# fakufaku/diffusion-separation

Hardware: AMD Instinct MI355X
Metric: separated utterances/sec (4 s, 8 kHz, 2-spk, N=30 PC steps) (higher is better)
Workload: dtype f16; 1 GPU; configs[1]: 2-spk N=30 PC sampler (+1 ald2 corrector step), batch=16 x 4.0 s @ 8 kHz per GPU and step, NCSN++ nf=64 random-init, 60 NFE/step; 4 consecutive steps (batches) in flight per GPU; batch_per_gpu=16, samples=32000, N=30, corrector_steps=1, nf=64, graph=True, batches_in_flight=4

## Files before the change

diffusion-separation_amd/csrc/common.h:

```cpp
#pragma once
#include <hip/hip_runtime.h>
#include <stdint.h>
#include <stdio.h>

#include <string>

typedef uint16_t bf16_t;
typedef __attribute__((ext_vector_type(16))) float f32x16;
typedef __attribute__((ext_vector_type(8))) __bf16 bf16x8;

#define DS_F32 0
#define DS_BF16 1
#define DS_F32_SPLIT 2
#define DS_MAX_SRC 4

void ds_set_error(const std::string& s);
#define DS_CHECK(cond, msg)                                                            \
  do {                                                                                 \
    if (!(cond)) {                                                                     \
      ds_set_error(std::string(__FILE__) + ":" + std::to_string(__LINE__) + ": " + (msg)); \
      return 1;                                                                        \
    }                                                                                  \
  } while (0)
#define DS_HIP(expr)                                                                   \
// ... 157 lines not shown
  const void* sw; int sw_chunked;
  const float* gn_scale;
  const float* gn_shift; int gn_act;
  const float* bias;
  const float* bias_b; int bias_b_ld;
  int bias_mode;
  const float* div_b;
  const void* res; long res_bs; int ldr;
  float out_scale;
  void* y; long y_bs; int ldy;
  long long* stats_acc;
  const long long* gn_acc1; const long long* gn_acc2; const float* gn_gamma; const float* gn_beta;
  int gn_groups; float gn_inv_count; float gn_eps;
  int B, H, W;
  int Cin, Cout, taps;
  int dtype;
  int split;
  unsigned opts;
};
#define DS_OPT_NO_RW 1u
#define DS_OPT_NO_RW128 2u
#define DS_OPT_RW_SMALL 4u
#define DS_OPT_NO_RW_RES 8u
#define DS_OPT_NO_ATTN_FUSED 64u
#define DS_OPT_NO_SPLIT256 128u
#define DS_OPT_NO_STFT_FUSED 256u
#define DS_OPT_RW_QUARTER 1024u
#define DS_OPT_RW_BIG_HALF 2048u
#define DS_OPT_RW_HALF 512u
#define DS_OPT_NO_SW 4096u
#define DS_OPT_NO_SW_RW 8192u
#define DS_OPT_NO_SW_ROWS4 32768u
#define DS_OPT_SW_ROWS4 65536u
#define DS_OPT_NO_SWS 16384u
#define DS_OPT_NO_WFRAG 32u
unsigned ds_default_opts();
int ds_num_cus();
enum { DS_CLS_CONV_N64 = 0, DS_CLS_CONV_N32, DS_CLS_CONV_8X8, DS_CLS_GEMM_N64, DS_CLS_GEMM_N32, DS_CLS_GEMM_8X8, DS_CLS_WS,
       DS_CLS_SMALL, DS_CLS_RW, DS_CLS_ATTN, DS_CLS_SW, DS_CLS_SWS, DS_NCLS };
enum class ConvRoute { GENERIC, WS, THIN_IN, THIN_OUT, SMALL, RW, SW, SWS };
struct ConvPlan {
  ConvRoute route;
  int cls;
  int tile;
  int sw_rows;
  bool rw_ok;
  bool skip_ok;
};
ConvPlan ds_conv_plan(const ConvArgs& a);
int ds_launch_conv(const ConvArgs& a, hipStream_t st);
int ds_launch_conv(const ConvArgs& a, const ConvPlan& p, hipStream_t st);
const char* ds_last_conv_kernel();
void ds_set_last_conv_kernel(const char* name);
int ds_conv_chunk(int taps, int dtype);
__host__ __device__ inline long ds_rw_frag_index(int co, int tap, int ch, int taps, int Cout) {
  return (((((long)(ch / 64) * taps + tap) * 4 + (ch % 64) / 16) * (Cout / 32) + co / 32) * 64 + ((ch % 16) / 8) * 32 + co % 32) * 8 + ch % 8;
}
inline bool ds_rw_frag_shape(int taps, int Cin, int Cout) {
  return (Cout == 64 || Cout == 128) && (Cin == 64 || Cin == 128) && (taps == 1 || !(Cout == 128 && Cin == 64));
}
bool ds_conv_rw_supported(const ConvArgs& a);
int ds_launch_conv_rw(const ConvArgs& a, hipStream_t st);
inline bool ds_sw_frag_shape(int taps, int Cin, int Cout) { return (Cout == 64 || Cout == 128 || Cout == 256) && Cin % 64 == 0 && Cin >= 64 && Cin <= 512; }
bool ds_conv_sw_supported(const ConvArgs& a);
int ds_launch_conv_sw(const ConvArgs& a, int rows, hipStream_t st);
__host__ __device__ inline long ds_sws_frag_index(int co, int tap, int ch, int taps, int Cout, int plane) {
  return ((((((long)(ch / 32) * taps + tap) * 2 + (ch % 32) / 16) * 2 + plane) * (Cout / 32) + co / 32) * 64 + ((ch % 16) / 8) * 32 + co % 32) * 8 + ch % 8;
}
inline bool ds_sws_frag_shape(int taps, int Cin, int Cout) { return (Cout == 64 || Cout == 128 || Cout == 256) && Cin % 64 == 0 && Cin >= 64 && Cin <= 256; }
bool ds_conv_sws_supported(const ConvArgs& a);
int ds_launch_conv_sws(const ConvArgs& a, hipStream_t st);
bool ds_conv_ws_supported(const ConvArgs& a);
int ds_launch_conv_ws(const ConvArgs& a, hipStream_t st);
bool ds_conv_thin_in_supported(const ConvArgs& a);
int ds_launch_conv_thin_in(const ConvArgs& a, hipStream_t st);
bool ds_conv_thin_out_supported(const ConvArgs& a);
int ds_launch_conv_thin_out(const ConvArgs& a, hipStream_t st);
bool ds_conv_small_supported(const ConvArgs& a);
int ds_launch_conv_small(const ConvArgs& a, hipStream_t st);

struct AttnFusedArgs {
  const void* x; long x_bs; int ldx;
  const long long* gn_acc; const float* gn_gamma; const float* gn_beta; int gn_groups; float gn_inv_count; float gn_eps;
  const float* gn_scale; const float* gn_shift;
  const void* wqk; const void* wv; const void* wo;
// ... 147 lines not shown
```

diffusion-separation_amd/csrc/conv3x3_halo.h:

```cpp
#pragma once

#include <ctype.h>
#include <stdlib.h>

#include <initializer_list>
#include <type_traits>

#include "conv_device.h"

#ifdef HALO_TIMING
#define HALO_CAT_(a, b, c) a##b##c
#define HALO_CAT(a, b, c) HALO_CAT_(a, b, c)
#define HALO_DBG HALO_CAT(g_, HALO_TIMING, _dbg)
__device__ unsigned long long HALO_DBG[16];
extern "C" int HALO_CAT(diffsep_, HALO_TIMING, _debug_read)(unsigned long long* out, int reset) {
  (void)hipMemcpyFromSymbol(out, HIP_SYMBOL(HALO_DBG), sizeof(unsigned long long) * 16);
  if (reset) { unsigned long long z[16] = {0}; (void)hipMemcpyToSymbol(HIP_SYMBOL(HALO_DBG), z, sizeof(z)); }
  return 0;
}
#define RT_DECL unsigned rt_prev = (unsigned)__builtin_readcyclecounter(), rt_acc[8] = {0, 0, 0, 0, 0, 0, 0, 0};
#define RT_MARK(i) { unsigned rt_now = (unsigned)__builtin_readcyclecounter(); rt_acc[i] += rt_now - rt_prev; rt_prev = rt_now; }
#define RT_FLUSH if (threadIdx.x == 0) { for (int q = 0; q < 8; ++q) atomicAdd(&HALO_DBG[q], (unsigned long long)rt_acc[q]); atomicAdd(&HALO_DBG[15], 1ull); }
#define HALO_STR_(a) #a
#define HALO_STR(a) HALO_STR_(a)
// ... 66 lines not shown
    k.sx2 = reinterpret_cast<const T*>(a.sx2); k.sx2_bs = a.sx2_bs; k.ldsx2 = a.sx2 ? a.ldsx2 : a.ldsx;
    k.swfrag = reinterpret_cast<const bf16_t*>(a.sw_frag);
    return a.sCin;
  }
  if (a.res) {
    k.sx = reinterpret_cast<const T*>(a.res); k.sx_bs = a.res_bs; k.ldsx = a.ldr; k.sC1 = a.Cout; k.ldsx2 = a.ldr;
    k.swfrag = reinterpret_cast<const bf16_t*>(a.ident_frag);
    return a.Cout;
  }
  return 0;
}

inline int halo_tiles(const ConvArgs& a, int tile_h) { return (a.H / tile_h) * (a.W / TW); }
inline int halo_blocks_wanted(const ConvArgs& a, int ncb) {
  const int g = ds_num_cus() / (a.B * ncb);
#ifdef HALO_TIMING
  return halo_env("G", g);
#else
  return g;
#endif
}
template <auto KERN, typename K>
int halo_launch(K k, const ConvArgs& a, int tile_h, int g, int ncb, int lds, hipStream_t st, const char* family,
                std::initializer_list<int> targs) {
  const int tiles = halo_tiles(a, tile_h);
  k.G = g < 1 ? 1 : (g > tiles ? tiles : g);
  k.tiles_x = a.W / TW;
  k.tiles_per_img = tiles;
  DS_FUNC_LDS_ONCE(KERN, lds);
  hipLaunchKernelGGL(KERN, dim3(a.B * ncb * k.G), dim3(NT), lds, st, k);
  DS_LAUNCH_CHECK();
  static char name[64] = {0};
  if (!name[0]) {
    char b[64];
    int n = snprintf(b, sizeof(b), "%s<", family);
    for (int v : targs) n += snprintf(b + n, sizeof(b) - n, "%d,", v);
    b[n - 1] = '>';
    for (int i = n; i >= 0; --i) name[i] = b[i];
  }
  ds_set_last_conv_kernel(name);
  return 0;
}

inline bool halo_concat_ok(const ConvArgs& a, int kc, int al) {
  return a.x2 ? a.C1 % kc == 0 && a.C1 > 0 && a.C1 < a.Cin && a.ldx % al == 0 && a.ldx2 % al == 0 : a.ldx % al == 0;
}
inline bool halo_gn_ok(const ConvArgs& a, int cpg_max) {
  if ((a.gn_scale || a.gn_acc1) && !a.gn_act) return false;
  return !a.gn_acc1 || (a.gn_groups > 0 && a.Cin % a.gn_groups == 0 && a.Cin / a.gn_groups <= cpg_max && (!a.x2 || a.gn_acc2));
}
inline bool halo_skip_split_ok(const ConvArgs& a, int kc, int al) {
  return a.ldsx % al == 0 && (!a.sx2 || (a.sC1 % kc == 0 && a.sC1 > 0 && a.sC1 < a.sCin && a.ldsx2 % al == 0));
}
// ... 16 lines not shown
```

diffusion-separation_amd/csrc/conv3x3_rw.hip:

```cpp
#include <stdlib.h>

#ifdef RW_TIMING
#define HALO_TIMING rw
#endif
#include "conv3x3_halo.h"

namespace {

constexpr int KC = 64;
constexpr int NKB = KC / 16;
constexpr int KSC = 9 * NKB;
static_assert(KC * 2 + 16 == AROW && KC / 8 == PPL, "a pixel's chunk is one 128-byte line");

struct RwK {
  const bf16_t* x; long x_bs; int ldx; int C1;
  const bf16_t* x2; long x2_bs; int ldx2;
  const bf16_t* w; int w_chunked;
  const bf16_t* wfrag; const bf16_t* swfrag;
  const float* gn_scale; const float* gn_shift;
  const long long* gn_acc1; const long long* gn_acc2; const float* gn_gamma; const float* gn_beta;
  int gn_groups; float gn_inv_count; float gn_eps;
  const float* bias; const float* bias_b; int bias_b_ld;
  const bf16_t* res; long res_bs; int ldr;
  float out_scale;
  bf16_t* y; long y_bs; int ldy;
  long long* stats;
  const bf16_t* sx; long sx_bs; int ldsx; int sC1;
  const bf16_t* sx2; long sx2_bs; int ldsx2;
  const bf16_t* sw; int sw_chunked; int sw_shift; int sCin;
  int H, W, G, tiles_x, tiles_per_img;
  int dbg;
};

#ifndef RW_NWL2
#define RW_NWL2 8
#endif
constexpr int rw_lds_ksteps(int nch, int rpw, int nsk, int ncg) { return ncg == 4 ? nch * KSC - 64 + nsk * NKB : (nch == 2 ? RW_NWL2 : 0); }

template <int NCH, int RPW, int NSK, int NCG>
struct RwGeom {
  static constexpr int CO = 32 * NCG, PGN = 4 / NCG;
  static constexpr int TH = PGN * RPW, HH_ = TH + 2, HP = HH_ * HW_;
  static constexpr int NI = TH * TW * PPL / NT, NBP = HP - TH * TW, NB = (NBP * PPL + NT - 1) / NT;
  static constexpr int NL = NI + NB;
  static_assert(NT / PPL == TW && TH * TW * PPL % NT == 0, "one staging pass = one tile row");
  static constexpr int LDS_A = NL * (NT / PPL) * AROW;
  static constexpr int CIN = NCH * KC, SCIN = NSK * KC;
  static constexpr int LDS_TAB = (2 * CIN + CO) * 4;
  static constexpr int LDS_DESC = NB * NT * 4;
  static_assert((NI + NB) * (NT / PPL) >= HP + NB * (NT / PPL) - NBP, "dummy pixels of the last border pass fit the slot");
  static constexpr int NPH = NCH + NSK;
  static constexpr int NKS = NCH * KSC + NSK * NKB;
  static constexpr int NWL = rw_lds_ksteps(NCH, RPW, NSK, NCG), NWR = NKS - NWL;
  static constexpr int LDS_WL = NWL * NCG * 64 * 16;
  static constexpr int WL_STEP = NCG * 64 * 16;
  static constexpr int OFF_TAB = 2 * LDS_A, OFF_WL = OFF_TAB + ((LDS_TAB + 15) & ~15), OFF_DESC = OFF_WL + LDS_WL;
  static constexpr int LDS_TOTAL = OFF_DESC + LDS_DESC;
  static constexpr int chunk_of(int P) { return P < NSK ? NCH + P : P - NSK; }
  static_assert(LDS_TOTAL <= 160 * 1024, "LDS budget of one CU");
  static_assert(NT * 36 * 4 <= LDS_TOTAL, "the statistics reduce reuses the block's LDS");
};

template <int NCH, int RPW, int NSK, int MODE, int NCG>
__global__ __launch_bounds__(NT, 1) void conv3x3_rw_kernel(RwK p) {
  using G = RwGeom<NCH, RPW, NSK, NCG>;
  constexpr int CO = G::CO, PGN = G::PGN;
  constexpr int TH = G::TH, HP = G::HP, LDS_A = G::LDS_A, NL = G::NL, NPH = G::NPH, NKS = G::NKS, CIN = G::CIN, NWR = G::NWR;
  extern __shared__ __attribute__((aligned(16))) char smem[];
  char* sA = smem;
  float* sTab = reinterpret_cast<float*>(smem + G::OFF_TAB);
  int* sDesc = reinterpret_cast<int*>(smem + G::OFF_DESC);
  const int tid = threadIdx.x;
  const int lane = tid & 63, wave = __builtin_amdgcn_readfirstlane(tid >> 6);
  const int l32 = lane & 31, h = lane >> 5;
  const int cg = wave % NCG, pg = wave / NCG;
  const int b = blockIdx.x / p.G, part = blockIdx.x % p.G;
  const int t0 = (int)((long)part * p.tiles_per_img / p.G);
  const int nt = (int)((long)(part + 1) * p.tiles_per_img / p.G) - t0;
  RT_DECL

  static_assert(CIN <= NT && CO <= NT, "one table entry per thread");
  constexpr int CPG_MAX = 8;
  long long t_s[CPG_MAX], t_q[CPG_MAX];
  float t_gam = 1.f, t_bet = 0.f, t_sc = 1.f, t_sh = 0.f, t_bias = 0.f;
#pragma unroll
  for (int j = 0; j < CPG_MAX; ++j) { t_s[j] = 0; t_q[j] = 0; }
  if (tid < CIN) {
    const int c = tid;
    if (p.gn_acc1) {
      const int C1 = p.C1, C2 = CIN - C1;
      const int cpg = CIN / p.gn_groups, g0 = (c / cpg) * cpg;
#pragma unroll
      for (int j = 0; j < CPG_MAX; ++j) {
        if (j < cpg) {
          const int cc = g0 + j;
          const long long* src = cc < C1 ? p.gn_acc1 + ((long)b * C1 + cc) * 2 : p.gn_acc2 + ((long)b * C2 + (cc - C1)) * 2;
          t_s[j] = src[0];
          t_q[j] = src[1];
        }
      }
      t_gam = p.gn_gamma ? p.gn_gamma[c] : 1.f;
      t_bet = p.gn_beta ? p.gn_beta[c] : 0.f;
    } else if (p.gn_scale) {
      t_sc = p.gn_scale[(long)b * CIN + c];
      t_sh = p.gn_shift[(long)b * CIN + c];
    }
  }
  if (tid < CO) t_bias = (p.bias ? p.bias[tid] : 0.f) + (p.bias_b ? p.bias_b[(long)b * p.bias_b_ld + tid] : 0.f);
  auto build_tables = [&]() __attribute__((always_inline)) {
    if (tid < CIN) {
      float sc = t_sc, sh = t_sh;
      if (p.gn_acc1) {
        long long t_ssum = 0, t_ssq = 0;
#pragma unroll
        for (int j = 0; j < CPG_MAX; ++j) { t_ssum += t_s[j]; t_ssq += t_q[j]; }
        ds_gn_affine_from_acc(t_ssum, t_ssq, p.gn_inv_count, p.gn_eps, t_gam, t_bet, sc, sh);
      }
      sTab[tid] = sc;
      sTab[CIN + tid] = sh;
    }
    if (tid < CO) sTab[2 * CIN + tid] = t_bias * p.out_scale;
  };
  const int slot = tid & (PPL - 1);
  constexpr int NI = G::NI, NB = G::NB, NBP = G::NBP;
  const int ixp = tid / PPL;
  unsigned fl = 0;
  int dstb[NB];
#pragma unroll
  for (int kb = 0; kb < NB; ++kb) {
    const int bi = ixp + (NT / PPL) * kb;
    int hy, hx;
// ... 206 lines not shown
#else
      if (P1 < NCH || k < NI)
        *reinterpret_cast<u32x4_t*>(sA + sl * LDS_A + (k < NI ? ldi0 + k * HW_ * AROW : dstb[k < NI ? 0 : k - NI])) = so;
#endif
#ifdef RW_ABL_NOLOAD
      pa[k][0] += rel;
#else
      issue_one(P2_, g2, k, rel);
#endif
    }
  };
  auto unit_s2 = [&](auto P1_, auto P2_, const TileG& g1, const TileG& g2, int sl, int u, int rel) __attribute__((always_inline)) {
    unit_s2x(P1_, P2_, std::false_type{}, g1, g2, sl, u, rel);
  };
  auto unit_fin = [&](auto P1_, auto P2_, const TileG& g1, const TileG& g2, int sl, int u, int rel) __attribute__((always_inline)) {
    unit_s2x(P1_, P2_, std::true_type{}, g1, g2, sl, u, rel);
  };
  auto unit = [&](auto P1_, auto P2_, const TileG& g1, const TileG& g2, int sl, int u, int rel) __attribute__((always_inline)) {
    unit_s01(P1_, u, -1);
    unit_s01(P1_, -1, u);
    unit_s2(P1_, P2_, g1, g2, sl, u, rel);
  };

  f32x16 acc[RPW];
#pragma unroll
  for (int r = 0; r < RPW; ++r)
#pragma unroll
    for (int e = 0; e < 16; ++e) acc[r][e] = 0.f;
  float ssum[16], ssq[16];
#pragma unroll
  for (int j = 0; j < 16; ++j) { ssum[j] = 0.f; ssq[j] = 0.f; }
  const bool has_stats = p.stats != nullptr;
  const float osc = FOLD ? p.out_scale * -0.6931471805599453f : p.out_scale;
  const int fbase = (pg * RPW * HW_ + l32) * AROW + h * 16;

  auto swap_halves = [&](u32x4_t& v) __attribute__((always_inline)) {
    auto r0 = __builtin_amdgcn_permlane32_swap(v.x, v.z, false, false);
    auto r1 = __builtin_amdgcn_permlane32_swap(v.y, v.w, false, false);
    v.x = r0[0]; v.z = r0[1]; v.y = r1[0]; v.w = r1[1];
  };
  u32x4_t ov0;
  const int srow = lane >> 4;
  const unsigned spiece = (unsigned)(cg * 64 + (srow & 1) * 32 + (srow >> 1) * 16);
  auto epi_unit = [&](const TileG& g, int r, int j, const float4& t0, const float4& t1) __attribute__((always_inline)) {
    float v[8];
    v[0] = fmaf(acc[r][8 * j + 0], osc, t0.x); v[1] = fmaf(acc[r][8 * j + 1], osc, t0.y);
// ... 58 lines not shown
  auto half = [&](auto P_, auto HF_, auto EPI_, int slot_r, const TileG& ge, const TileG& g1, const TileG& g2) __attribute__((always_inline)) {
    constexpr int P = decltype(P_)::value, HF = decltype(HF_)::value;
    constexpr bool EPI = decltype(EPI_)::value;
    constexpr int C = G::chunk_of(P);
    constexpr bool CONV = C < NCH;
    constexpr int NK = CONV ? KSC : NKB;
    constexpr int W0 = CONV ? C * KSC : NCH * KSC + (C - NCH) * NKB;
    constexpr int C1 = G::chunk_of((P + 1) % NPH), C2 = G::chunk_of((P + 2) % NPH);
    constexpr int NU = NL * 4;
    constexpr bool ACT1 = C1 < NCH && MODE != 0;
    constexpr int LAG = ACT1 ? PIPE_LAG : 0, NUV = NU + LAG, NLU = 2 * NUV;
    constexpr int NGH = NK * RH;
    constexpr int w0 = (P == 0) ? W_E : W_N, w1 = (P == NPH - 1) ? W_E : W_N, CAP = NGH * (w0 + w1);
    auto lub = [](int GP) constexpr { return NLU * (GP <= NGH ? GP * w0 : NGH * w0 + (GP - NGH) * w1) / CAP; };
    constexpr int NLE = RH * 22;
    constexpr int R0 = HF * RH, ER0 = HF ? 0 : RH;
    const char* fb = sA + slot_r * LDS_A + fbase + R0 * HW_ * AROW;
#ifndef RW_BUILTIN_MFMA
    if constexpr (EPI) {
#pragma unroll
      for (int r = 0; r < RH; ++r) asm volatile("s_nop 11" : "+v"(acc[ER0 + r]));
    }
#endif
    if constexpr (HF == 0 && C1 < NCH) act_tab(C1);
    constexpr int SUB = CONV ? 3 : 1, RFN = CONV ? RH + 2 : RH, NG = NK / SUB;
    static_assert(SUB * RH >= RFN, "the next group's fragments are read in the MFMA slots of the current one");
    auto ldg = [&](int g, int j) __attribute__((always_inline)) {
      const int dx = CONV ? g / NKB : 1, kb = g % NKB, row = CONV ? j : j + 1;
      return *reinterpret_cast<const u32x4_t*>(fb + (row * HW_ + dx) * AROW + kb * 32);
    };
    u32x4_t rf[2][RFN];
#pragma unroll
    for (int j = 0; j < RFN; ++j) rf[0][j] = ldg(0, j);
    auto widx = [](int ks) {
      if (!CONV) return ks;
      const int g = ks / 3, dy = ks % 3, dx = g / NKB, kb = g % NKB;
      return (dy * 3 + dx) * NKB + kb;
    };
#define RW_FRAG(ks, r) rf[((ks) / SUB) & 1][(r) + (CONV ? (ks) % SUB : 0)]
#define RW_FRAG_LAST(ks) rf[((ks) / SUB) & 1][RFN - 1]
    u32x4_t wl = {0, 0, 0, 0}, wln = {0, 0, 0, 0};
    if constexpr (W0 + widx(0) >= NWR) wl = *reinterpret_cast<const u32x4_t*>(sWl + (W0 + widx(0) - NWR) * G::WL_STEP);
    int rels[2][NL];
    auto fetch_rels = [&](int ks, int par) __attribute__((always_inline)) {
      const int gp0 = HF * NGH + ks * RH;
#pragma unroll
      for (int L = lub(gp0); L < lub(gp0 + RH); ++L) {
        const int u = (L >> 1) - LAG;
        if ((L & 1) && u >= 0 && u < NU && (u & 3) == 3 && (u >> 2) >= NI)
          rels[par][u >> 2] = REL_REGS ? relreg[(u >> 2) - NI] : sDesc[((u >> 2) - NI) * NT + tid];
      }
    };
    fetch_rels(0, 0);

    auto unit_lump = [&](int L, int par) __attribute__((always_inline)) {
      const int v = L >> 1;
      const int u0 = v < NU ? v : -1, u1 = LAG ? ((v >= 1 && v - 1 < NU) ? v - 1 : -1) : v, u2 = v - LAG;
      const bool s2 = u2 >= 0 && u2 < NU;
      if ((L & 1) == 0) {
        if constexpr (ACT1 && ACT_PK) {
          if (u0 >= 0) {
            asm volatile("v_pk_fma_f16 %0, %1, %2, %3" : "=v"(uzp[u0 % 3]) : "v"(pa[u0 >> 2][u0 & 3]), "v"(psc[u0 & 3]), "v"(psh[u0 & 3]));
            if constexpr (MODE == 2 && !FOLD) asm volatile("v_pk_mul_f16 %0, %1, %2" : "=v"(uxp[u0 % 3]) : "v"(uzp[u0 % 3]), "s"(0xbdc5bdc5u));
          }
          if constexpr (MODE == 2) {
            if (u1 >= 0) asm volatile("v_pk_add_f16 %0, %1, %2" : "=v"(udp[u1 % 3]) : "v"(utp[u1 % 3]), "s"(0x3c003c00u));
            if (s2) asm volatile("v_pk_mul_f16 %0, %1, %2" : "=v"(so[u2 & 3]) : "v"(uzp[u2 % 3]), "v"(urp[u2 % 3]));
            if (u0 >= 0) asm volatile("v_exp_f16 %0, %1" : "=v"(utp[u0 % 3]) : "v"(FOLD ? uzp[u0 % 3] : uxp[u0 % 3]));
            if (u1 >= 0) asm volatile("v_rcp_f16 %0, %1" : "=v"(urp[u1 % 3]) : "v"(udp[u1 % 3]));
          } else {
            if (s2) so[u2 & 3] = uzp[u2 % 3];
          }
        } else if constexpr (ACT1) {
          if (u0 >= 0) unit_s01(std::integral_constant<int, C1>{}, u0, -1);
        }
      } else {
// ... 52 lines not shown
        }
      } else if (x == 20) {
#pragma unroll
        for (int d = 0; d < 4; ++d) asm volatile("v_permlane16_swap_b32 %0, %1" : "+v"(osa[d]), "+v"(osb[d]));
      } else {
        const int pix = ge.pix0 + (pg * RPW + rr) * p.W + (lane & 15);
        const unsigned o = __umul24((unsigned)pix, (unsigned)p.ldy * 2u) + spiece;
#ifdef RW_TIMING
        const unsigned o1 = (p.dbg & 1) ? OOB : o, o2 = (p.dbg & 1) ? OOB : o + 16u * (unsigned)p.ldy * 2u;
#else
        const unsigned o1 = o, o2 = o + 16u * (unsigned)p.ldy * 2u;
#endif
#ifdef RW_ABL_NOSTORE
        asm volatile("" :: "v"(osa), "v"(osb), "v"(o1), "v"(o2));
#else
        __builtin_amdgcn_raw_buffer_store_b128(osa, ry, o1, 0, 0);
        __builtin_amdgcn_raw_buffer_store_b128(osb, ry, o2, 0, 0);
#endif
      }
    };

#pragma unroll
    for (int ks = 0; ks < NK; ++ks) {
      if (ks + 1 < NK) fetch_rels(ks + 1, (ks + 1) & 1);
      const int wi = W0 + widx(ks), win = W0 + widx(ks + 1 < NK ? ks + 1 : ks);
      if (win >= NWR && ks + 1 < NK) wln = *reinterpret_cast<const u32x4_t*>(sWl + (win - NWR) * G::WL_STEP);
      const u32x4_t wk = wi < NWR ? wf[wi < NWR ? wi : 0] : wl;
#define RW_DEP , "v"(RW_FRAG_LAST(ks))
#pragma unroll
      for (int r = 0; r < RH; ++r) {
        if (wi < NWR) {
          if (P == 0 && ks == 0) asm volatile(DS_MFMA_H32_ASM " %0, %1, %2, 0" : "=v"(acc[R0 + r]) : "a"(wk), "v"(RW_FRAG(ks, r)) RW_DEP);
          else asm volatile(DS_MFMA_H32_ASM " %0, %1, %2, %0" : "+v"(acc[R0 + r]) : "a"(wk), "v"(RW_FRAG(ks, r)) RW_DEP);
        } else {
          if (P == 0 && ks == 0) asm volatile(DS_MFMA_H32_ASM " %0, %1, %2, 0" : "=v"(acc[R0 + r]) : "v"(wk), "v"(RW_FRAG(ks, r)) RW_DEP);
          else asm volatile(DS_MFMA_H32_ASM " %0, %1, %2, %0" : "+v"(acc[R0 + r]) : "v"(wk), "v"(RW_FRAG(ks, r)) RW_DEP);
        }
        {
          const int g = ks / SUB, q = (ks % SUB) * RH + r;
          if (q < RFN && g + 1 < NG) rf[(g + 1) & 1][q] = ldg(g + 1, q);
        }
        const int gh = ks * RH + r, gp = HF * NGH + gh;
#pragma unroll
        for (int L = lub(gp); L < lub(gp + 1); ++L) unit_lump(L, ks & 1);
#ifndef RW_ABL_NOEPI
        if constexpr (EPI) {
#pragma unroll
          for (int LE = gh * NLE / NGH; LE < (gh + 1) * NLE / NGH; ++LE) epi_lump(LE);
        }
#endif
      }
      wl = wln;
      __builtin_amdgcn_sched_barrier(0);
    }
  };

  TileG gc = tile_geom(0);
  constexpr int CH0 = G::chunk_of(0), CH1 = G::chunk_of(1 % NPH);
  const TileG g1st = NPH > 1 ? gc : tile_geom(1);
  {
#pragma unroll
    for (int k = 0; k < NL; ++k) issue_one(std::integral_constant<int, CH0>{}, gc, k, k < NI ? 0 : sDesc[(k < NI ? 0 : k - NI) * NT + tid]);
    load_weights();
    build_tables();
    sync_lds();
    RT_MARK(7)
    if constexpr (REL_REGS) {
#pragma unroll
      for (int k = 0; k < NB; ++k) relreg[k] = sDesc[k * NT + tid];
    }
    if constexpr (BIAS_REGS) {
#pragma unroll
      for (int j = 0; j < 2; ++j) {
        breg[j][0] = *reinterpret_cast<const float4*>(sTab + 2 * CIN + cg * 32 + 8 * (2 * j) + 4 * h);
        breg[j][1] = *reinterpret_cast<const float4*>(sTab + 2 * CIN + cg * 32 + 8 * (2 * j + 1) + 4 * h);
      }
    }
    act_tab(CH0);
#pragma unroll
    for (int u = 0; u < NL * 4; ++u)
      unit(std::integral_constant<int, CH0>{}, std::integral_constant<int, CH1>{}, gc, g1st, 0, u,
           (u >> 2) < NI ? 0 : sDesc[((u >> 2) < NI ? 0 : (u >> 2) - NI) * NT + tid]);
  }
  RT_MARK(0)
  TileG gp = tile_geom(nt);
  int ph = 0;
  TileG gnc = tile_geom(1);
  int ty2 = (t0 + 2) / p.tiles_x, tx2 = (t0 + 2) - ty2 * p.tiles_x;
  for (int i = 0; i < nt; ++i) {
    const TileG gn = gnc, gnn = geom_at(ty2, tx2, i + 2 < nt);
    auto run = [&](auto self, auto P_) __attribute__((always_inline)) {
      constexpr int P = decltype(P_)::value;
      sync_lds();
      RT_MARK(1)
      const int slot_r = ph & 1;
      half(P_, std::integral_constant<int, 0>{}, std::integral_constant<bool, P == 0>{}, slot_r, gp, ((P + 1) / NPH == 0 ? gc : gn), ((P + 2) / NPH == 0 ? gc : ((P + 2) / NPH == 1 ? gn : gnn)));
      if constexpr (P == 0) {
        if (i == 0) {
#pragma unroll
          for (int j = 0; j < 16; ++j) { ssum[j] = 0.f; ssq[j] = 0.f; }
        }
      }
      half(P_, std::integral_constant<int, 1>{}, std::integral_constant<bool, P == NPH - 1>{}, slot_r, gc, ((P + 1) / NPH == 0 ? gc : gn), ((P + 2) / NPH == 0 ? gc : ((P + 2) / NPH == 1 ? gn : gnn)));
      ++ph;
      RT_MARK(G::chunk_of(P) < NCH ? 2 : 3)
// ... 32 lines not shown
      double a = 0.0;
      for (int wpg = 0; wpg < PGN; ++wpg)
        for (int l = 0; l < 32; ++l) {
          const int t = (wpg * NCG + wcg) * 64 + hh * 32 + l;
          a += (double)red[t * RED_ROW + st * 16 + 4 * q + i];
        }
      ds_stat_flush(p.stats + ((long)b * CO + co) * 2, st, a);
    }
  }
  RT_MARK(5)
  RT_FLUSH
}

int rw_blocks_per_image(const ConvArgs& a, int tiles) {
  int g = halo_blocks_wanted(a, 1);
  if ((a.opts & DS_OPT_RW_HALF) && g >= 2 && tiles / g <= 4) g /= 2;
  if ((a.opts & DS_OPT_RW_QUARTER) && g >= 4 && tiles / g <= 4) g /= 4;
  if ((a.opts & DS_OPT_RW_BIG_HALF) && g >= 2 && tiles / g > 4) g /= 2;
  return g;
}

template <int NCH, int RPW, int NSK, int MODE, int NCG>
int rw_launch(const RwK& k, const ConvArgs& a, hipStream_t st) {
  using G = RwGeom<NCH, RPW, NSK, NCG>;
  static_assert(G::TH <= HALO_TH_MAX, "halo_addressing_ok covers the tile");
  return halo_launch<conv3x3_rw_kernel<NCH, RPW, NSK, MODE, NCG>>(k, a, G::TH, rw_blocks_per_image(a, halo_tiles(a, G::TH)), 1, G::LDS_TOTAL, st,
                                                                 "conv3x3_rw_kernel", {NCH, RPW, NSK, MODE, NCG});
}

#define RW_SHAPES(X)                                                                        \
  X(64, 1, 0, 0) X(64, 1, 1, 0) X(64, 1, 2, 0) X(64, 1, 3, 0) X(64, 2, 0, 0)                \
  X(64, 1, 0, 2) X(64, 1, 1, 2) X(64, 1, 2, 2) X(64, 1, 3, 2) X(64, 2, 0, 2)                \
  X(128, 2, 0, 0) X(128, 2, 0, 2) X(128, 2, 1, 2) X(128, 2, 2, 2)
#define RW_IS(CO_, NCH_, NSK_, MODE_) cout == CO_ && nch == NCH_ && nsk == NSK_ && mode == MODE_
bool rw_shape(int cout, int nch, int nsk, int mode) {
#define RW_CASE(CO_, NCH_, NSK_, MODE_) if (RW_IS(CO_, NCH_, NSK_, MODE_)) return true;
  RW_SHAPES(RW_CASE)
#undef RW_CASE
  return false;
}
int rw_dispatch(const RwK& k, const ConvArgs& a, int cout, int nch, int nsk, int mode, hipStream_t st) {
#define RW_CASE(CO_, NCH_, NSK_, MODE_) if (RW_IS(CO_, NCH_, NSK_, MODE_)) return rw_launch<NCH_, 4, NSK_, MODE_, CO_ / 32>(k, a, st);
  RW_SHAPES(RW_CASE)
#undef RW_CASE
  return -1;
}
#undef RW_IS

}

bool ds_conv_rw_supported(const ConvArgs& a) {
  const int CO = a.Cout;
  if (!(a.dtype == DS_BF16 && a.taps == 9 && a.Cin % KC == 0 && a.w_bs == 0 && (a.w_chunked == 0 || a.w_chunked == 32) &&
        a.bias_mode == 0 && !a.div_b && a.W % TW == 0 && a.H % 8 == 0 && a.H >= 32 && a.W >= 32 && a.ldy >= CO && a.ldy % 8 == 0 &&
        (!a.res || (a.ldr >= CO && a.ldr % 8 == 0))))
    return false;
  if (!halo_concat_ok(a, KC, 8) || !halo_gn_ok(a, 8) || !halo_addressing_ok(a, 2, true)) return false;
  int nsk = 0;
  if (a.sx) {
    if (!(a.sw && !a.res && a.sCin % KC == 0 && a.sCin >= KC && halo_skip_split_ok(a, KC, 8) &&
          (a.sw_chunked == 0 || ((a.sw_chunked & (a.sw_chunked - 1)) == 0 && a.sw_chunked >= 16))))
      return false;
    nsk = a.sCin / KC;
  } else if (a.res) {
    nsk = CO / KC;
  }
  return rw_shape(CO, a.Cin / KC, nsk, (a.gn_scale || a.gn_acc1) ? 2 : 0);
}

int ds_launch_conv_rw(const ConvArgs& a, hipStream_t st) {
  RwK k;
  halo_fill_common(k, a);
  k.w = reinterpret_cast<const bf16_t*>(a.w); k.w_chunked = a.w_chunked;
  k.wfrag = reinterpret_cast<const bf16_t*>(a.w_frag);
  k.swfrag = (a.sx && a.sw) ? reinterpret_cast<const bf16_t*>(a.sw_frag) : nullptr;
  k.res = reinterpret_cast<const bf16_t*>(a.res); k.res_bs = a.res_bs; k.ldr = a.ldr;
  k.sx = reinterpret_cast<const bf16_t*>(a.sx); k.sx_bs = a.sx_bs; k.ldsx = a.ldsx; k.sC1 = a.sx2 ? a.sC1 : a.sCin;
  k.sx2 = reinterpret_cast<const bf16_t*>(a.sx2); k.sx2_bs = a.sx2_bs; k.ldsx2 = a.sx2 ? a.ldsx2 : a.ldsx;
  k.sw = reinterpret_cast<const bf16_t*>(a.sw); k.sw_chunked = a.sw_chunked; k.sw_shift = a.sw_chunked ? __builtin_ctz(a.sw_chunked) : 0;
  k.sCin = a.sCin;
  if (a.res) {
    k.sx = reinterpret_cast<const bf16_t*>(a.res); k.sx_bs = a.res_bs; k.ldsx = a.ldr; k.sC1 = a.Cout;
    k.sx2 = nullptr; k.sx2_bs = 0; k.ldsx2 = a.ldr; k.sw = nullptr; k.sw_chunked = 0; k.sw_shift = 0; k.sCin = a.Cout;
  }
  const int mode = ((a.gn_scale || a.gn_acc1) && a.gn_act) ? 2 : 0;
  const int nsk = a.sx ? a.sCin / KC : (a.res ? a.Cout / KC : 0);
  const int rc = rw_dispatch(k, a, a.Cout, a.Cin / KC, nsk, mode, st);
  DS_CHECK(rc >= 0, "conv3x3_rw: shape outside the instantiated set");
  return rc;
}
```

diffusion-separation_amd/csrc/engine.hip:

```cpp
#include "engine_host.h"

static thread_local std::string g_err;
void ds_set_error(const std::string& s) { g_err = s; }
extern "C" const char* diffsep_last_error(void) { return g_err.c_str(); }
extern "C" const char* diffsep_version(void) {
#ifdef DS_HALF_F16
    return "diffsep-hip 0.3 (gfx950, 16-bit storage f16)";
#else
    return "diffsep-hip 0.3 (gfx950, 16-bit storage bf16)";
#endif
}

static const struct { const char* name; const char* env; unsigned bit; } kOpts[] = {
    {"no_rw", "DIFFSEP_NO_RW", DS_OPT_NO_RW},
    {"no_rw128", "DIFFSEP_NO_RW128", DS_OPT_NO_RW128},
    {"rw_small", "DIFFSEP_RW_SMALL", DS_OPT_RW_SMALL},
    {"no_rw_res", "DIFFSEP_NO_RW_RES", DS_OPT_NO_RW_RES},
    {"no_wfrag", nullptr, DS_OPT_NO_WFRAG},
    {"no_attn_fused", nullptr, DS_OPT_NO_ATTN_FUSED},
    {"no_stft_fused", "DIFFSEP_NO_STFT_FUSED", DS_OPT_NO_STFT_FUSED},
    {"rw_half", "DIFFSEP_RW_HALF", DS_OPT_RW_HALF},
    {"rw_quarter", "DIFFSEP_RW_QUARTER", DS_OPT_RW_QUARTER},
    {"rw_big_half", "DIFFSEP_RW_BIG_HALF", DS_OPT_RW_BIG_HALF},
    {"no_split256", nullptr, DS_OPT_NO_SPLIT256},
    {"no_sw", "DIFFSEP_NO_SW", DS_OPT_NO_SW},
    {"no_sws", "DIFFSEP_NO_SWS", DS_OPT_NO_SWS},
    {"no_sw_rows4", "DIFFSEP_NO_SW_ROWS4", DS_OPT_NO_SW_ROWS4},
    {"sw_rows4", nullptr, DS_OPT_SW_ROWS4},
    {"no_sw_rw", "DIFFSEP_NO_SW_RW", DS_OPT_NO_SW_RW}};
static std::atomic<unsigned> g_opts{0};
static std::once_flag g_opts_once;
unsigned ds_default_opts() {
  std::call_once(g_opts_once, [] {
    for (const auto& o : kOpts) {
      const char* v = o.env ? getenv(o.env) : nullptr;
      if (v && *v && strcmp(v, "0") != 0) g_opts |= o.bit;
    }
  });
  return g_opts;
}
// ... 832 lines not shown
```

Before: 77.75 utterances/s.

## Add helper-wave warp specialization to RW conv for GN-activated 64-channel shapes

```diff
diff --git a/diffusion-separation_amd/csrc/common.h b/diffusion-separation_amd/csrc/common.h
--- a/diffusion-separation_amd/csrc/common.h
+++ b/diffusion-separation_amd/csrc/common.h
@@ -203,6 +203,7 @@
 #define DS_OPT_NO_RW128 2u
 #define DS_OPT_RW_SMALL 4u
 #define DS_OPT_NO_RW_RES 8u
+#define DS_OPT_NO_RW_HELPER 131072u
 #define DS_OPT_NO_ATTN_FUSED 64u
 #define DS_OPT_NO_SPLIT256 128u
 #define DS_OPT_NO_STFT_FUSED 256u
@@ -242,6 +243,7 @@
 }
 bool ds_conv_rw_supported(const ConvArgs& a);
 int ds_launch_conv_rw(const ConvArgs& a, hipStream_t st);
+int ds_launch_conv_rw4(const ConvArgs& a, hipStream_t st);
 inline bool ds_sw_frag_shape(int taps, int Cin, int Cout) { return (Cout == 64 || Cout == 128 || Cout == 256) && Cin % 64 == 0 && Cin >= 64 && Cin <= 512; }
 bool ds_conv_sw_supported(const ConvArgs& a);
 int ds_launch_conv_sw(const ConvArgs& a, int rows, hipStream_t st);
diff --git a/diffusion-separation_amd/csrc/conv3x3_halo.h b/diffusion-separation_amd/csrc/conv3x3_halo.h
--- a/diffusion-separation_amd/csrc/conv3x3_halo.h
+++ b/diffusion-separation_amd/csrc/conv3x3_halo.h
@@ -112,13 +112,13 @@
 }
 template <auto KERN, typename K>
 int halo_launch(K k, const ConvArgs& a, int tile_h, int g, int ncb, int lds, hipStream_t st, const char* family,
-                std::initializer_list<int> targs) {
+                std::initializer_list<int> targs, int threads = NT) {
   const int tiles = halo_tiles(a, tile_h);
   k.G = g < 1 ? 1 : (g > tiles ? tiles : g);
   k.tiles_x = a.W / TW;
   k.tiles_per_img = tiles;
   DS_FUNC_LDS_ONCE(KERN, lds);
-  hipLaunchKernelGGL(KERN, dim3(a.B * ncb * k.G), dim3(NT), lds, st, k);
+  hipLaunchKernelGGL(KERN, dim3(a.B * ncb * k.G), dim3(threads), lds, st, k);
   DS_LAUNCH_CHECK();
   static char name[64] = {0};
   if (!name[0]) {
diff --git a/diffusion-separation_amd/csrc/conv3x3_rw.hip b/diffusion-separation_amd/csrc/conv3x3_rw.hip
--- a/diffusion-separation_amd/csrc/conv3x3_rw.hip
+++ b/diffusion-separation_amd/csrc/conv3x3_rw.hip
@@ -1,7 +1,11 @@
 #include <stdlib.h>
 
 #ifdef RW_TIMING
+#ifdef RW_FOUR_WAVE_TU
+#define HALO_TIMING rw4
+#else
 #define HALO_TIMING rw
+#endif
 #endif
 #include "conv3x3_halo.h"
 
@@ -37,7 +41,18 @@
 #endif
 constexpr int rw_lds_ksteps(int nch, int rpw, int nsk, int ncg) { return ncg == 4 ? nch * KSC - 64 + nsk * NKB : (nch == 2 ? RW_NWL2 : 0); }
 
-template <int NCH, int RPW, int NSK, int NCG>
+#ifndef RW_HELPER_WREGS
+#define RW_HELPER_WREGS 20
+#endif
+constexpr bool rw_helper_form(int nch, int mode, int ncg) {
+#ifdef RW_NO_HELPER
+  return false;
+#else
+  return nch == 1 && mode == 2 && ncg == 2;
+#endif
+}
+
+template <int NCH, int RPW, int NSK, int NCG, bool HLP = false>
 struct RwGeom {
   static constexpr int CO = 32 * NCG, PGN = 4 / NCG;
   static constexpr int TH = PGN * RPW, HH_ = TH + 2, HP = HH_ * HW_;
@@ -51,7 +66,7 @@
   static_assert((NI + NB) * (NT / PPL) >= HP + NB * (NT / PPL) - NBP, "dummy pixels of the last border pass fit the slot");
   static constexpr int NPH = NCH + NSK;
   static constexpr int NKS = NCH * KSC + NSK * NKB;
-  static constexpr int NWL = rw_lds_ksteps(NCH, RPW, NSK, NCG), NWR = NKS - NWL;
+  static constexpr int NWL = HLP ? NKS - RW_HELPER_WREGS : rw_lds_ksteps(NCH, RPW, NSK, NCG), NWR = NKS - NWL;
   static constexpr int LDS_WL = NWL * NCG * 64 * 16;
   static constexpr int WL_STEP = NCG * 64 * 16;
   static constexpr int OFF_TAB = 2 * LDS_A, OFF_WL = OFF_TAB + ((LDS_TAB + 15) & ~15), OFF_DESC = OFF_WL + LDS_WL;
@@ -62,15 +77,20 @@
 };
 
 template <int NCH, int RPW, int NSK, int MODE, int NCG>
-__global__ __launch_bounds__(NT, 1) void conv3x3_rw_kernel(RwK p) {
-  using G = RwGeom<NCH, RPW, NSK, NCG>;
+__global__ __launch_bounds__(rw_helper_form(NCH, MODE, NCG) ? 2 * NT : NT, rw_helper_form(NCH, MODE, NCG) ? 2 : 1) void conv3x3_rw_kernel(RwK p) {
+  constexpr bool HLP = rw_helper_form(NCH, MODE, NCG);
+  using G = RwGeom<NCH, RPW, NSK, NCG, HLP>;
   constexpr int CO = G::CO, PGN = G::PGN;
   constexpr int TH = G::TH, HP = G::HP, LDS_A = G::LDS_A, NL = G::NL, NPH = G::NPH, NKS = G::NKS, CIN = G::CIN, NWR = G::NWR;
   extern __shared__ __attribute__((aligned(16))) char smem[];
   char* sA = smem;
   float* sTab = reinterpret_cast<float*>(smem + G::OFF_TAB);
   int* sDesc = reinterpret_cast<int*>(smem + G::OFF_DESC);
-  const int tid = threadIdx.x;
+  const int tid = HLP ? (int)(threadIdx.x & (NT - 1)) : (int)threadIdx.x;
+  const bool helper = HLP && __builtin_amdgcn_readfirstlane((int)threadIdx.x >> 8) != 0;
+  constexpr int BAR_PRO_M = 1, BAR_PH_M = 1, BAR_TAIL_M = 2;
+  constexpr int BAR_PRO_H = 1, BAR_PH_H = 1, BAR_TAIL_H = 2;
+  static_assert(BAR_PRO_M == BAR_PRO_H && BAR_PH_M == BAR_PH_H && BAR_TAIL_M == BAR_TAIL_H, "both roles meet at every barrier");
   const int lane = tid & 63, wave = __builtin_amdgcn_readfirstlane(tid >> 6);
   const int l32 = lane & 31, h = lane >> 5;
   const int cg = wave % NCG, pg = wave / NCG;
@@ -85,7 +105,7 @@
   float t_gam = 1.f, t_bet = 0.f, t_sc = 1.f, t_sh = 0.f, t_bias = 0.f;
 #pragma unroll
   for (int j = 0; j < CPG_MAX; ++j) { t_s[j] = 0; t_q[j] = 0; }
-  if (tid < CIN) {
+  if (!helper && tid < CIN) {
     const int c = tid;
     if (p.gn_acc1) {
       const int C1 = p.C1, C2 = CIN - C1;
@@ -106,7 +126,7 @@
       t_sh = p.gn_shift[(long)b * CIN + c];
     }
   }
-  if (tid < CO) t_bias = (p.bias ? p.bias[tid] : 0.f) + (p.bias_b ? p.bias_b[(long)b * p.bias_b_ld + tid] : 0.f);
+  if (!helper && tid < CO) t_bias = (p.bias ? p.bias[tid] : 0.f) + (p.bias_b ? p.bias_b[(long)b * p.bias_b_ld + tid] : 0.f);
   auto build_tables = [&]() __attribute__((always_inline)) {
     if (tid < CIN) {
       float sc = t_sc, sh = t_sh;
@@ -359,6 +379,170 @@
     unit_s2(P1_, P2_, g1, g2, sl, u, rel);
   };
 
+  if constexpr (HLP && NSK > 0) {
+    if (helper) {
+      using C0 = std::integral_constant<int, 0>;
+      u32x4_t ps[NI];
+      auto issue_skip = [&](auto C_, const TileG& g, int k) __attribute__((always_inline)) {
+        constexpr int CB = (decltype(C_)::value - NCH) * KC;
+        const bool second = CB >= p.sC1;
+        const unsigned ld2 = (unsigned)(second ? p.ldsx2 : p.ldsx) * 2u;
+        const unsigned co2 = (unsigned)((second ? CB - p.sC1 : CB) * 2) + (unsigned)slot * 16u;
+        ps[k] = ld16v(second ? rs2 : rs1, __umul24((unsigned)(g.pix0 + k * p.W + ixp), ld2) + co2, 0);
+      };
+      auto put_skip = [&](int sl, int k) __attribute__((always_inline)) {
+        *reinterpret_cast<u32x4_t*>(sA + sl * LDS_A + ldi0 + k * HW_ * AROW) = ps[k];
+      };
+      auto act_inplace = [&](int u) __attribute__((always_inline)) {
+        unit_s01(C0{}, u, -1);
+        unit_s01(C0{}, -1, u);
+        const int k = u >> 2, d = u & 3, q = u % 3;
+        if constexpr (ACT_PK) {
+          unsigned v;
+          asm volatile("v_pk_mul_f16 %0, %1, %2" : "=v"(v) : "v"(uzp[q]), "v"(urp[q]));
+          so[d] = v;
+        } else {
+          so[d] = pack_h2(uz[q][0] * ut[q][0], uz[q][1] * ut[q][1]);
+        }
+        if (d == 3) pa[k] = so;
+      };
+      auto put_conv = [&](const TileG& g1, const TileG& g2, int sl, int k, int rel) __attribute__((always_inline)) {
+        so = pa[k];
+        if (k >= NI) {
+          const bool ok = piece_ok(C0{}, g1, k);
+          so.x = ok ? so.x : 0u;
+          so.y = ok ? so.y : 0u;
+          so.z = ok ? so.z : 0u;
+          so.w = ok ? so.w : 0u;
+        }
+        *reinterpret_cast<u32x4_t*>(sA + sl * LDS_A + (k < NI ? ldi0 + k * HW_ * AROW : dstb[k < NI ? 0 : k - NI])) = so;
+        issue_one(C0{}, g2, k, rel);
+      };
+      TileG hc = tile_geom(0);
+      TileG hnc = tile_geom(1);
+      int hrel[NB];
+#pragma unroll
+      for (int k = 0; k < NB; ++k) hrel[k] = sDesc[k * NT + tid];
+#pragma unroll
+      for (int k = 0; k < NI; ++k) issue_skip(std::integral_constant<int, NCH>{}, hc, k);
+#pragma unroll
+      for (int k = 0; k < NL; ++k) issue_one(C0{}, hc, k, k < NI ? 0 : hrel[k < NI ? 0 : k - NI]);
+      sync_lds();
+      RT_MARK(0)
+#pragma unroll
+      for (int k = 0; k < NI; ++k) {
+        put_skip(0, k);
+        if constexpr (NSK > 1) issue_skip(std::integral_constant<int, NCH + 1>{}, hc, k);
+        else issue_skip(std::integral_constant<int, NCH>{}, hnc, k);
+      }
+      act_tab(0);
+#pragma unroll
+      for (int u = 0; u < NL * 4; ++u) act_inplace(u);
+      RT_MARK(1)
+      int hph = 0;
+      int hy2 = (t0 + 2) / p.tiles_x, hx2 = (t0 + 2) - hy2 * p.tiles_x;
+      for (int i = 0; i < nt; ++i) {
+        const TileG hn = hnc, hnn = geom_at(hy2, hx2, i + 2 < nt);
+        auto stage_phase = [&](auto self, auto P_) __attribute__((always_inline)) {
+          constexpr int P = decltype(P_)::value;
+          sync_lds();
+          RT_MARK(2)
+          const int sl = (hph & 1) ^ 1;
+          if constexpr (P == NSK - 1) {
+#pragma unroll
+            for (int k = 0; k < NL; ++k) put_conv(hc, hn, sl, k, k < NI ? 0 : hrel[k < NI ? 0 : k - NI]);
+          } else {
+            constexpr int SW = (P + 1) % NPH;
+            constexpr bool NEXT = P == NSK, WRAP = SW + 1 >= NSK;
+            constexpr int SN = WRAP ? 0 : SW + 1;
+            const TileG& gsn = NEXT ? (WRAP ? hnn : hn) : (WRAP ? hn : hc);
+#pragma unroll
+            for (int k = 0; k < NI; ++k) {
+              put_skip(sl, k);
+              issue_skip(std::integral_constant<int, NCH + SN>{}, gsn, k);
+            }
+            if constexpr (P == NSK) {
+#pragma unroll
+              for (int u = 0; u < NL * 4; ++u) act_inplace(u);
+            }
+          }
+          ++hph;
+          RT_MARK(3)
+          if constexpr (P + 1 < NPH) self(self, std::integral_constant<int, P + 1>{});
+        };
+        stage_phase(stage_phase, std::integral_constant<int, 0>{});
+        hc = hn;
+        hnc = hnn;
+        if (++hx2 == p.tiles_x) { hx2 = 0; ++hy2; }
+      }
+      if (p.stats != nullptr) {
+        __syncthreads();
+        __syncthreads();
+      }
+#ifdef RW_TIMING
+      if (threadIdx.x == NT) {
+        for (int q = 0; q < 4; ++q) atomicAdd(&HALO_DBG[8 + q], (unsigned long long)rt_acc[q]);
+      }
+#endif
+      return;
+    }
+  }
+  if constexpr (HLP && NSK == 0) {
+    if (helper) {
+      constexpr int HC0 = G::chunk_of(0), HC1 = G::chunk_of(1 % NPH);
+      TileG hc = tile_geom(0);
+      const TileG h1st = NPH > 1 ? hc : tile_geom(1);
+#pragma unroll
+      for (int k = 0; k < NL; ++k) issue_one(std::integral_constant<int, HC0>{}, hc, k, k < NI ? 0 : sDesc[(k < NI ? 0 : k - NI) * NT + tid]);
+      int hrel[NB];
+#pragma unroll
+      for (int k = 0; k < NB; ++k) hrel[k] = sDesc[k * NT + tid];
+      sync_lds();
+      RT_MARK(0)
+      act_tab(HC0);
+#pragma unroll
+      for (int u = 0; u < NL * 4; ++u)
+        unit(std::integral_constant<int, HC0>{}, std::integral_constant<int, HC1>{}, hc, h1st, 0, u, (u >> 2) < NI ? 0 : hrel[(u >> 2) < NI ? 0 : (u >> 2) - NI]);
+      RT_MARK(1)
+      int hph = 0;
+      TileG hnc = tile_geom(1);
+      int hy2 = (t0 + 2) / p.tiles_x, hx2 = (t0 + 2) - hy2 * p.tiles_x;
+      for (int i = 0; i < nt; ++i) {
+        const TileG hn = hnc, hnn = geom_at(hy2, hx2, i + 2 < nt);
+        auto stage_phase = [&](auto self, auto P_) __attribute__((always_inline)) {
+          constexpr int P = decltype(P_)::value;
+          constexpr int C1 = G::chunk_of((P + 1) % NPH), C2 = G::chunk_of((P + 2) % NPH);
+          sync_lds();
+          RT_MARK(2)
+          const int sl = (hph & 1) ^ 1;
+          const TileG& g1 = (P + 1) / NPH == 0 ? hc : hn;
+          const TileG& g2 = (P + 2) / NPH == 0 ? hc : ((P + 2) / NPH == 1 ? hn : hnn);
+          if constexpr (C1 < NCH) act_tab(C1);
+#pragma unroll
+          for (int u = 0; u < NL * 4; ++u)
+            unit(std::integral_constant<int, C1>{}, std::integral_constant<int, C2>{}, g1, g2, sl, u, (u >> 2) < NI ? 0 : hrel[(u >> 2) < NI ? 0 : (u >> 2) - NI]);
+          ++hph;
+          RT_MARK(3)
+          if constexpr (P + 1 < NPH) self(self, std::integral_constant<int, P + 1>{});
+        };
+        stage_phase(stage_phase, std::integral_constant<int, 0>{});
+        hc = hn;
+        hnc = hnn;
+        if (++hx2 == p.tiles_x) { hx2 = 0; ++hy2; }
+      }
+      if (p.stats != nullptr) {
+        __syncthreads();
+        __syncthreads();
+      }
+#ifdef RW_TIMING
+      if (threadIdx.x == NT) {
+        for (int q = 0; q < 4; ++q) atomicAdd(&HALO_DBG[8 + q], (unsigned long long)rt_acc[q]);
+      }
+#endif
+      return;
+    }
+  }
+
   f32x16 acc[RPW];
 #pragma unroll
   for (int r = 0; r < RPW; ++r)
@@ -463,7 +647,7 @@
       for (int r = 0; r < RH; ++r) asm volatile("s_nop 11" : "+v"(acc[ER0 + r]));
     }
 #endif
-    if constexpr (HF == 0 && C1 < NCH) act_tab(C1);
+    if constexpr (!HLP && HF == 0 && C1 < NCH) act_tab(C1);
     constexpr int SUB = CONV ? 3 : 1, RFN = CONV ? RH + 2 : RH, NG = NK / SUB;
     static_assert(SUB * RH >= RFN, "the next group's fragments are read in the MFMA slots of the current one");
     auto ldg = [&](int g, int j) __attribute__((always_inline)) {
@@ -492,7 +676,7 @@
           rels[par][u >> 2] = REL_REGS ? relreg[(u >> 2) - NI] : sDesc[((u >> 2) - NI) * NT + tid];
       }
     };
-    fetch_rels(0, 0);
+    if constexpr (!HLP) fetch_rels(0, 0);
 
     auto unit_lump = [&](int L, int par) __attribute__((always_inline)) {
       const int v = L >> 1;
@@ -591,14 +775,16 @@
 
 #pragma unroll
     for (int ks = 0; ks < NK; ++ks) {
-      if (ks + 1 < NK) fetch_rels(ks + 1, (ks + 1) & 1);
+      if constexpr (!HLP) {
+        if (ks + 1 < NK) fetch_rels(ks + 1, (ks + 1) & 1);
+      }
       const int wi = W0 + widx(ks), win = W0 + widx(ks + 1 < NK ? ks + 1 : ks);
       if (win >= NWR && ks + 1 < NK) wln = *reinterpret_cast<const u32x4_t*>(sWl + (win - NWR) * G::WL_STEP);
       const u32x4_t wk = wi < NWR ? wf[wi < NWR ? wi : 0] : wl;
 #define RW_DEP , "v"(RW_FRAG_LAST(ks))
 #pragma unroll
       for (int r = 0; r < RH; ++r) {
-        if (wi < NWR) {
+        if (!HLP && wi < NWR) {
           if (P == 0 && ks == 0) asm volatile(DS_MFMA_H32_ASM " %0, %1, %2, 0" : "=v"(acc[R0 + r]) : "a"(wk), "v"(RW_FRAG(ks, r)) RW_DEP);
           else asm volatile(DS_MFMA_H32_ASM " %0, %1, %2, %0" : "+v"(acc[R0 + r]) : "a"(wk), "v"(RW_FRAG(ks, r)) RW_DEP);
         } else {
@@ -610,8 +796,10 @@
           if (q < RFN && g + 1 < NG) rf[(g + 1) & 1][q] = ldg(g + 1, q);
         }
         const int gh = ks * RH + r, gp = HF * NGH + gh;
-#pragma unroll
-        for (int L = lub(gp); L < lub(gp + 1); ++L) unit_lump(L, ks & 1);
+        if constexpr (!HLP) {
+#pragma unroll
+          for (int L = lub(gp); L < lub(gp + 1); ++L) unit_lump(L, ks & 1);
+        }
 #ifndef RW_ABL_NOEPI
         if constexpr (EPI) {
 #pragma unroll
@@ -628,13 +816,15 @@
   constexpr int CH0 = G::chunk_of(0), CH1 = G::chunk_of(1 % NPH);
   const TileG g1st = NPH > 1 ? gc : tile_geom(1);
   {
-#pragma unroll
-    for (int k = 0; k < NL; ++k) issue_one(std::integral_constant<int, CH0>{}, gc, k, k < NI ? 0 : sDesc[(k < NI ? 0 : k - NI) * NT + tid]);
+    if constexpr (!HLP) {
+#pragma unroll
+      for (int k = 0; k < NL; ++k) issue_one(std::integral_constant<int, CH0>{}, gc, k, k < NI ? 0 : sDesc[(k < NI ? 0 : k - NI) * NT + tid]);
+    }
     load_weights();
     build_tables();
     sync_lds();
     RT_MARK(7)
-    if constexpr (REL_REGS) {
+    if constexpr (REL_REGS && !HLP) {
 #pragma unroll
       for (int k = 0; k < NB; ++k) relreg[k] = sDesc[k * NT + tid];
     }
@@ -645,11 +835,13 @@
         breg[j][1] = *reinterpret_cast<const float4*>(sTab + 2 * CIN + cg * 32 + 8 * (2 * j + 1) + 4 * h);
       }
     }
-    act_tab(CH0);
-#pragma unroll
-    for (int u = 0; u < NL * 4; ++u)
-      unit(std::integral_constant<int, CH0>{}, std::integral_constant<int, CH1>{}, gc, g1st, 0, u,
-           (u >> 2) < NI ? 0 : sDesc[((u >> 2) < NI ? 0 : (u >> 2) - NI) * NT + tid]);
+    if constexpr (!HLP) {
+      act_tab(CH0);
+#pragma unroll
+      for (int u = 0; u < NL * 4; ++u)
+        unit(std::integral_constant<int, CH0>{}, std::integral_constant<int, CH1>{}, gc, g1st, 0, u,
+             (u >> 2) < NI ? 0 : sDesc[((u >> 2) < NI ? 0 : (u >> 2) - NI) * NT + tid]);
+    }
   }
   RT_MARK(0)
   TileG gp = tile_geom(nt);
@@ -728,16 +920,21 @@
 
 template <int NCH, int RPW, int NSK, int MODE, int NCG>
 int rw_launch(const RwK& k, const ConvArgs& a, hipStream_t st) {
-  using G = RwGeom<NCH, RPW, NSK, NCG>;
+  constexpr bool HLP = rw_helper_form(NCH, MODE, NCG);
+  using G = RwGeom<NCH, RPW, NSK, NCG, HLP>;
   static_assert(G::TH <= HALO_TH_MAX, "halo_addressing_ok covers the tile");
   return halo_launch<conv3x3_rw_kernel<NCH, RPW, NSK, MODE, NCG>>(k, a, G::TH, rw_blocks_per_image(a, halo_tiles(a, G::TH)), 1, G::LDS_TOTAL, st,
-                                                                 "conv3x3_rw_kernel", {NCH, RPW, NSK, MODE, NCG});
+                                                                 "conv3x3_rw_kernel", {NCH, RPW, NSK, MODE, NCG}, HLP ? 2 * NT : NT);
 }
 
+#ifdef RW_FOUR_WAVE_TU
+#define RW_SHAPES(X) X(64, 1, 0, 2) X(64, 1, 1, 2) X(64, 1, 2, 2) X(64, 1, 3, 2)
+#else
 #define RW_SHAPES(X)                                                                        \
   X(64, 1, 0, 0) X(64, 1, 1, 0) X(64, 1, 2, 0) X(64, 1, 3, 0) X(64, 2, 0, 0)                \
   X(64, 1, 0, 2) X(64, 1, 1, 2) X(64, 1, 2, 2) X(64, 1, 3, 2) X(64, 2, 0, 2)                \
   X(128, 2, 0, 0) X(128, 2, 0, 2) X(128, 2, 1, 2) X(128, 2, 2, 2)
+#endif
 #define RW_IS(CO_, NCH_, NSK_, MODE_) cout == CO_ && nch == NCH_ && nsk == NSK_ && mode == MODE_
 bool rw_shape(int cout, int nch, int nsk, int mode) {
 #define RW_CASE(CO_, NCH_, NSK_, MODE_) if (RW_IS(CO_, NCH_, NSK_, MODE_)) return true;
@@ -755,6 +952,9 @@
 
 }
 
+#ifdef RW_FOUR_WAVE_TU
+#define ds_launch_conv_rw ds_launch_conv_rw4
+#else
 bool ds_conv_rw_supported(const ConvArgs& a) {
   const int CO = a.Cout;
   if (!(a.dtype == DS_BF16 && a.taps == 9 && a.Cin % KC == 0 && a.w_bs == 0 && (a.w_chunked == 0 || a.w_chunked == 32) &&
@@ -773,8 +973,13 @@
   }
   return rw_shape(CO, a.Cin / KC, nsk, (a.gn_scale || a.gn_acc1) ? 2 : 0);
 }
+#endif
 
 int ds_launch_conv_rw(const ConvArgs& a, hipStream_t st) {
+#ifndef RW_FOUR_WAVE_TU
+  if ((a.opts & DS_OPT_NO_RW_HELPER) && rw_helper_form(a.Cin / KC, ((a.gn_scale || a.gn_acc1) && a.gn_act) ? 2 : 0, a.Cout / 32))
+    return ds_launch_conv_rw4(a, st);
+#endif
   RwK k;
   halo_fill_common(k, a);
   k.w = reinterpret_cast<const bf16_t*>(a.w); k.w_chunked = a.w_chunked;
diff --git a/diffusion-separation_amd/csrc/conv3x3_rw4.hip b/diffusion-separation_amd/csrc/conv3x3_rw4.hip
--- /dev/null
+++ b/diffusion-separation_amd/csrc/conv3x3_rw4.hip
@@ -0,0 +1,3 @@
+#define RW_NO_HELPER
+#define RW_FOUR_WAVE_TU
+#include "conv3x3_rw.hip"
diff --git a/diffusion-separation_amd/csrc/engine.hip b/diffusion-separation_amd/csrc/engine.hip
--- a/diffusion-separation_amd/csrc/engine.hip
+++ b/diffusion-separation_amd/csrc/engine.hip
@@ -16,6 +16,7 @@
     {"no_rw128", "DIFFSEP_NO_RW128", DS_OPT_NO_RW128},
     {"rw_small", "DIFFSEP_RW_SMALL", DS_OPT_RW_SMALL},
     {"no_rw_res", "DIFFSEP_NO_RW_RES", DS_OPT_NO_RW_RES},
+    {"no_rw_helper", nullptr, DS_OPT_NO_RW_HELPER},
     {"no_wfrag", nullptr, DS_OPT_NO_WFRAG},
     {"no_attn_fused", nullptr, DS_OPT_NO_ATTN_FUSED},
     {"no_stft_fused", "DIFFSEP_NO_STFT_FUSED", DS_OPT_NO_STFT_FUSED},
```

After: 79.14 utterances/s (median of 6 runs). +1.8%, better.
